# LiWentomng/OrientedRepPoints

Measured on AMD Instinct MI355X. Metric: images/sec (1024x1024 DOTA, R-50 FPN), higher is better.
Workload: dtype f32; 1 GPU; configs[1]: OrientedRepPoints R-50 FPN inference, 1024x1024 patch, 15 classes, bs=1/GPU, nms_pre=2000, score_thr=0.05, rnms iou_thr=0.4, max_per_img=2000; random-init weights, head biases calibrated to ~2000 dets/img; global_batch=1, parallelism=replicas x1 (image-parallel, no collective), images_in_flight_per_gpu=4

## Files before the change

### include/orp_hip.h

```cpp
#ifndef ORP_HIP_H_
#define ORP_HIP_H_

#include <stddef.h>
#include <stdint.h>

#ifdef __cplusplus
extern "C" {
#endif

#define ORP_OK 0
#define ORP_EINVAL (-1)
#define ORP_EWORKSPACE (-2)
#define ORP_ETOOBIG (-3)

const char* orp_version(void);

#define ORP_NMS_MAX_BOXES 131072
size_t orp_rnms_workspace_bytes(int n);
int orp_rnms(const float* dets, int n, float iou_thr, int flavor, int presorted, int order_out,
             int64_t* keep_out, int32_t* num_keep, void* workspace, size_t workspace_bytes, void* stream);

size_t orp_rnms_batched_workspace_bytes(int n_total, int nseg, int max_seg);
int orp_rnms_batched(const float* dets, int n_total, const int32_t* seg_offsets, int nseg, int max_seg,
                     float iou_thr, int flavor, int64_t* keep_out, int32_t* num_keep,
// ... 226 lines not shown
int orp_fpn_topdown_nhwc(const orp_norm_level* levels, const float* const* gammas_host, const float* const* betas_host,
                         int nlevels, int batch, int channels, int groups, float eps, uint32_t* amax_out, void* workspace,
                         size_t workspace_bytes, void* stream);

typedef struct { const float* input; const float* residual; float* output; float* output2; int height; int width; } orp_bias_level;
int orp_bias_act_multi(const orp_bias_level* levels_host, int nlevels, int batch, int channels, const float* bias,
                       const float* sub, int relu, void* stream);

size_t orp_conv1x1_packed_floats(int c_in);
int orp_conv1x1_ok(int c_in, int c_out);
int orp_conv1x1_pack_weight(const float* weight, int c_out, int c_in, float* packed, void* stream);
int orp_conv1x1_multi(const orp_bias_level* levels_host, int nlevels, int batch, int c_in, int c_out,
                      const float* weight_packed, const float* bias, const float* sub, int relu, void* stream);

int orp_conv1x1_bn_act_ok(int c_in, int c_out);
int orp_conv1x1_bn_act_pays(int c_in, int c_out, int hw, int batch, int has_residual);
int orp_conv1x1_bn_act_tile(int c_in, int c_out, int hw, int batch, int* tile_channels, int* tile_positions);
int orp_conv1x1_bn_act(const float* x, const float* weight_t, const float* scale, const float* shift, const float* residual,
                       const float* scale2, const float* shift2, float* y, int batch, int c_in, int c_out, int hw, int relu,
                       void* stream);

int orp_conv1x1_bn_act_range(const float* x, const float* weight_t, const float* scale, const float* shift, const float* residual,
                             const float* scale2, const float* shift2, float* y, int batch, int c_in, int c_out, int hw, int relu,
                             uint32_t* range_out, void* stream);
int orp_conv1x1_bn_act_pieces_ok(int c_in, int c_out);
int orp_conv1x1_bn_act_pieces_pays(int c_in, int c_out, int hw, int batch, int has_residual);
int orp_conv1x1_bn_act_pieces_tile(int c_in, int c_out, int hw, int batch, int* tile_channels, int* tile_positions);
size_t orp_conv1x1_bn_pieces_packed_bytes(int c_in, int c_out);
int orp_conv1x1_bn_pieces_pack_weight(const float* weight, int c_in, int c_out, void* packed, void* stream);
int orp_conv1x1_bn_act_pieces(const float* x, const void* weight_packed, const float* scale, const float* shift,
                              const float* residual, const float* scale2, const float* shift2, float* y, int batch, int c_in,
                              int c_out, int hw, int relu, uint32_t* range_out, void* stream);

int orp_conv1x1_bn_act_pieces_dual_ok(int c_in, int c_in2, int c_out);
int orp_conv1x1_bn_act_pieces_dual_pays(int c_in, int c_in2, int c_out, int hw, int stride2, int batch);
int orp_conv1x1_bn_act_pieces_dual_tile(int c_in, int c_in2, int c_out, int hw, int batch, int* tile_channels, int* tile_positions);
int orp_conv1x1_bn_act_pieces_dual(const float* x, const void* w_packed, const float* scale, const float* shift, const float* x2,
                                   const void* w2_packed, const float* scale2, const float* shift2, int c_in2, int h2, int w2,
                                   int stride2, float* y, int batch, int c_in, int c_out, int ho, int wo, int relu, void* stream);

int orp_affine_act_range(const float* x, const float* residual, const float* scale, const float* shift, float* y, int batch,
                         int channels, int hw, int relu, uint32_t* range_out, void* stream);

int orp_conv3x3_bn_act_ok(int c_in, int c_out);
int orp_conv3x3_bn_act_pays(int c_in, int c_out, int height, int width, int batch);
int orp_conv3x3_bn_act_tile(int c_in, int c_out, int height, int width, int batch, int* tile_h, int* tile_w, int* waves_pos,
                            int* waves_ch);
size_t orp_conv3x3_bn_packed_bytes(int c_in, int c_out);
int orp_conv3x3_bn_pack_weight(const float* weight, int c_in, int c_out, void* packed, void* stream);
int orp_conv3x3_bn_act(const float* x, const void* weight_packed, const float* scale, const float* shift, const uint32_t* range_in,
                       float* y, int batch, int c_in, int c_out, int height, int width, int relu, void* stream);

int orp_conv3x3_bn_deep_ok(int c_in, int c_out, int stride);
int orp_conv3x3_bn_deep_pays(int c_in, int c_out, int height, int width, int stride, int batch);
size_t orp_conv3x3_bn_deep_packed_bytes(int c_in, int c_out);
int orp_conv3x3_bn_deep_pack_weight(const float* weight, int c_in, int c_out, void* packed, void* stream);
int orp_conv3x3_bn_deep(const float* x, const void* weight_packed, const float* scale, const float* shift, const uint32_t* range_in,
                        float* y, int batch, int c_in, int c_out, int height, int width, int stride, int relu, void* stream);


int orp_conv3x3_small_ok(int c_in, int c_out);
int orp_conv3x3_small_multi(const orp_norm_level* levels_host, int nlevels, int batch, int c_in, int c_out,
                            const float* weight_packed, void* stream);
int orp_conv3x3_small_multi_ex(const orp_norm_level* levels_host, const float* const* weights_packed_host, int nlevels,
                               int batch, int c_in, int c_out, void* stream);
size_t orp_conv3x3_small_workspace_bytes(const orp_norm_level* levels_host, const int* strides_host, int nlevels, int batch,
// ... 94 lines not shown
```

### orientedreppoints_amd/_lib.py

```python
import ctypes
import os

import torch

_HERE = os.path.dirname(os.path.abspath(__file__))
LIB_PATH = os.environ.get("ORP_HIP_LIB") or os.path.join(_HERE, "csrc", "liborp_hip.so")

ORP_OK, ORP_EINVAL, ORP_EWORKSPACE, ORP_ETOOBIG = 0, -1, -2, -3
ORP_NMS_MAX_BOXES = 131072

_vp = ctypes.c_void_p
_i = ctypes.c_int
_f = ctypes.c_float
_sz = ctypes.c_size_t

_SIGNATURES = {
    "orp_version": (ctypes.c_char_p, []),
    "orp_rnms_workspace_bytes": (_sz, [_i]),
    "orp_rnms": (_i, [_vp, _i, _f, _i, _i, _i, _vp, _vp, _vp, _sz, _vp]),
    "orp_rnms_batched_workspace_bytes": (_sz, [_i, _i, _i]),
    "orp_rnms_batched": (_i, [_vp, _i, _vp, _i, _i, _f, _i, _vp, _vp, _vp, _sz, _vp]),
    "_poly_nms": (None, [_vp, _vp, _vp, _i, _i, _f, _i]),
    "_overlaps": (None, [_vp, _vp, _vp, _i, _i, _i]),
    "orp_quad_iou_matrix": (_i, [_vp, _i, _vp, _i, _i, _i, _vp, _vp]),
# ... 57 lines not shown
    "orp_poly_nms_f64_workspace_bytes": (_sz, [_i]),
    "orp_poly_nms_f64": (_i, [_vp, _i, ctypes.c_double, _vp, _vp, _vp, _sz, _vp]),
    "orp_poly_nms_f64_batched_workspace_bytes": (_sz, [_i, _i, _i]),
    "orp_poly_nms_f64_batched": (_i, [_vp, _i, _vp, _i, _i, ctypes.c_double, _i, _i, _vp, _vp, _vp, _sz, _vp]),
    "orp_scene_tiles": (_i, [_vp, _i, _i, ctypes.c_longlong, _vp, _i, _i, _vp, _vp, _i, _i, _vp, _vp]),
    "orp_scene_tiles_resized": (_i, [_vp, _i, _i, ctypes.c_longlong, _vp, _i, _i, _i, _i, _i, _i, _i, _vp, _vp, _vp, _vp, _vp, _vp, _i,
                                     _i, _vp, _vp]),
    "orp_scene_tiles_flip": (_i, [_vp, _i, _i, ctypes.c_longlong, _vp, _i, _i, _vp, _vp, _i, _i, _vp, _vp]),
    "orp_scene_tiles_resized_flip": (_i, [_vp, _i, _i, ctypes.c_longlong, _vp, _i, _i, _i, _i, _i, _i, _i, _vp, _vp, _vp, _vp, _vp,
                                          _vp, _i, _i, _vp, _vp]),
    "orp_scene_collect_workspace_bytes": (_sz, [_i, _i]),
    "orp_scene_collect": (_i, [_vp, _i, _i, _vp, ctypes.c_double, _i, _i, _vp, _vp, _vp, _vp, _vp, _sz, _vp]),
    "orp_soft_rnms_host": (_i, [_vp, _i, _f, _i, _f, _f, _vp, _vp]),
    "orp_conv1x1_packed_floats": (_sz, [_i]),
    "orp_conv1x1_ok": (_i, [_i, _i]),
    "orp_conv1x1_pack_weight": (_i, [_vp, _i, _i, _vp, _vp]),
    "orp_conv1x1_multi": (_i, [_vp, _i, _i, _i, _i, _vp, _vp, _vp, _i, _vp]),
    "orp_conv1x1_bn_act_ok": (_i, [_i, _i]),
    "orp_conv1x1_bn_act_pays": (_i, [_i, _i, _i, _i, _i]),
    "orp_conv1x1_bn_act_tile": (_i, [_i, _i, _i, _i, _vp, _vp]),
    "orp_conv1x1_bn_act": (_i, [_vp, _vp, _vp, _vp, _vp, _vp, _vp, _vp, _i, _i, _i, _i, _i, _vp]),
    "orp_conv1x1_bn_act_range": (_i, [_vp, _vp, _vp, _vp, _vp, _vp, _vp, _vp, _i, _i, _i, _i, _i, _vp, _vp]),
    "orp_affine_act_range": (_i, [_vp, _vp, _vp, _vp, _vp, _i, _i, _i, _i, _vp, _vp]),
    "orp_conv1x1_bn_act_pieces_ok": (_i, [_i, _i]),
    "orp_conv1x1_bn_act_pieces_pays": (_i, [_i, _i, _i, _i, _i]),
    "orp_conv1x1_bn_act_pieces_tile": (_i, [_i, _i, _i, _i, _vp, _vp]),
    "orp_conv1x1_bn_pieces_packed_bytes": (_sz, [_i, _i]),
    "orp_conv1x1_bn_pieces_pack_weight": (_i, [_vp, _i, _i, _vp, _vp]),
    "orp_conv1x1_bn_act_pieces": (_i, [_vp, _vp, _vp, _vp, _vp, _vp, _vp, _vp, _i, _i, _i, _i, _i, _vp, _vp]),
    "orp_conv1x1_bn_act_pieces_dual_ok": (_i, [_i, _i, _i]),
    "orp_conv1x1_bn_act_pieces_dual_pays": (_i, [_i, _i, _i, _i, _i, _i]),
    "orp_conv1x1_bn_act_pieces_dual_tile": (_i, [_i, _i, _i, _i, _i, _vp, _vp]),
    "orp_conv1x1_bn_act_pieces_dual": (_i, [_vp, _vp, _vp, _vp, _vp, _vp, _vp, _vp, _i, _i, _i, _i, _vp, _i, _i, _i, _i, _i, _i, _vp]),
    "orp_conv3x3_bn_act_ok": (_i, [_i, _i]),
    "orp_conv3x3_bn_act_pays": (_i, [_i, _i, _i, _i, _i]),
    "orp_conv3x3_bn_act_tile": (_i, [_i, _i, _i, _i, _i, _vp, _vp, _vp, _vp]),
    "orp_conv3x3_bn_packed_bytes": (_sz, [_i, _i]),
    "orp_conv3x3_bn_pack_weight": (_i, [_vp, _i, _i, _vp, _vp]),
    "orp_conv3x3_bn_act": (_i, [_vp, _vp, _vp, _vp, _vp, _vp, _i, _i, _i, _i, _i, _i, _vp]),
    "orp_conv3x3_bn_deep_ok": (_i, [_i, _i, _i]),
    "orp_conv3x3_bn_deep_pays": (_i, [_i, _i, _i, _i, _i, _i]),
    "orp_conv3x3_bn_deep_packed_bytes": (_sz, [_i, _i]),
    "orp_conv3x3_bn_deep_pack_weight": (_i, [_vp, _i, _i, _vp, _vp]),
    "orp_conv3x3_bn_deep": (_i, [_vp, _vp, _vp, _vp, _vp, _vp, _i, _i, _i, _i, _i, _i, _i, _vp]),
    "orp_pp_select_scratch_bytes": (_sz, [_i, _i, _i]),
    "orp_pp_select": (_i, [_vp, _i, _i, _vp, _i, _i, _vp, _vp, _sz, _vp]),
    "orp_pp_gather": (_i, [_vp, _vp, _i, _i, _vp, _vp, _vp, _i, _vp, _vp, _vp, _vp, _vp]),
    "orp_pp_compact_scratch_bytes": (_sz, [_i]),
    "orp_pp_compact": (_i, [_vp, _vp, _i, _i, _i, _vp, _f, _i, _vp, _vp, _vp, _vp, _vp, _vp, _sz, _vp]),
    "orp_pp_compact_views_scratch_bytes": (_sz, [_i]),
    "orp_pp_compact_views": (_i, [_vp, _i, _i, _f, _i, _vp, _vp, _vp, _vp, _vp, _vp, _vp, _vp, _sz, _vp]),
    "orp_pp_pack": (_i, [_vp, _vp, _vp, _vp, _vp, _vp, _vp, _vp, _i, _i, _vp, _vp]),
    "orp_groupnorm_workspace_bytes": (_sz, [_vp, _i, _i, _i, _i]),
    "orp_groupnorm_act_multi": (_i, [_vp, _i, _i, _i, _i, _vp, _vp, _f, _i, _vp, _sz, _vp]),
    "orp_groupnorm_act_multi_ex": (_i, [_vp, _vp, _vp, _i, _i, _i, _i, _f, _i, _vp, _sz, _vp]),
    "orp_groupnorm_act_multi_nhwc": (_i, [_vp, _vp, _vp, _vp, _i, _i, _i, _i, _f, _i, _vp, _sz, _vp]),
    "orp_groupnorm_act_multi_train": (_i, [_vp, _vp, _vp, _i, _i, _i, _i, _f, _i, _vp, _vp, _sz, _vp]),
    "orp_groupnorm_backward_workspace_bytes": (_sz, [_vp, _i, _i, _i, _i]),
    "orp_groupnorm_act_multi_backward": (_i, [_vp, _vp, _vp, _vp, _vp, _vp, _vp, _i, _i, _i, _i, _i, _vp, _vp, _sz, _vp]),
    "orp_voc_best_match_f64": (_i, [_vp, _vp, _i, _vp, _vp, _i, _vp, _vp, _vp]),
    "orp_affine_act": (_i, [_vp, _vp, _vp, _vp, _vp, _i, _i, _i, _i, _vp]),
    "orp_affine2_act": (_i, [_vp, _vp, _vp, _vp, _vp, _vp, _vp, _i, _i, _i, _i, _vp]),
    "orp_affine_relu_maxpool": (_i, [_vp, _vp, _vp, _vp, _i, _i, _i, _i, _vp]),
    "orp_fpn_topdown_workspace_bytes": (_sz, [_vp, _i, _i, _i, _i]),
    "orp_fpn_topdown_nhwc": (_i, [_vp, _vp, _vp, _i, _i, _i, _i, _f, _vp, _vp, _sz, _vp]),
    "orp_bias_act_multi": (_i, [_vp, _i, _i, _i, _vp, _vp, _i, _vp]),
# ... 105 lines not shown
```

### orientedreppoints_amd/build.py

```python
import concurrent.futures
import os
import subprocess

HERE = os.path.dirname(os.path.abspath(__file__))
CSRC = os.path.join(HERE, "csrc")
LIB = os.path.join(CSRC, "liborp_hip.so")
HIPCC = os.environ.get("HIPCC", "/opt/rocm/bin/hipcc")
ARCH = "gfx950"

NO_PACKED_FP32 = ["-Xclang", "-target-feature", "-Xclang", "-packed-fp32-ops"]
COMMON = ["--offload-arch=" + ARCH, "-O3", "-std=c++17", "-fPIC", "-Wall", "-Wno-unused-function",
          "-Wno-unused-result", "-Wno-unused-value",
          "-Wno-bitwise-instead-of-logical"]
if os.environ.get("ORP_PACKED_FP32", "0") != "1":
    COMMON = COMMON + NO_PACKED_FP32
SOURCES = [
    ("orp_nms.hip", ["-ffp-contract=off"]),
    ("orp_overlaps.hip", ["-ffp-contract=off"]),
    ("orp_minarearect.hip", ["-ffp-contract=off"]),
    ("orp_box_iou_rotated.hip", ["-ffp-contract=off"]),
    ("orp_convex.hip", ["-ffp-contract=off"]),
    ("orp_convex_giou.hip", ["-ffp-contract=off"]),
    ("orp_pointwise.hip", ["-ffp-contract=off"]),
    ("orp_assign.hip", ["-ffp-contract=off"]),
    ("orp_postproc.hip", ["-ffp-contract=off"]),
    ("orp_soft_rnms.hip", ["-ffp-contract=off"]),
    ("orp_scene.hip", ["-ffp-contract=off"]),
    ("orp_eval.hip", ["-ffp-contract=off"]),
    ("orp_train.hip", ["-ffp-contract=off"]),
    ("orp_norm.hip", []),
    ("orp_conv_small.hip", []),
    ("orp_conv1x1.hip", []),
    ("orp_conv1x1_bn.hip", []),
    ("orp_conv1x1_bn_pieces.hip", []),
    ("orp_conv3x3_bn.hip", []),
    ("orp_conv3x3_bn_deep.hip", []),
    ("orp_dcn.hip", []),
    ("orp_dcn_split.hip", ["-ffp-contract=off"]),
    ("orp_conv_split.hip", []),
    ("orp_conv_wgrad.hip", []),
    ("orp_dcn_half.hip", []),
    ("orp_dcn_bwd.hip", []),
    ("orp_dcn_bwd_mfma.hip", []),
    ("orp_window_attn.hip", []),
    ("orp_prof.hip", []),
]
HEADERS = ["orp_affine.hpp", "orp_geom.hpp", "orp_quadfast.hpp", "orp_tile.hpp", "orp_hull.hpp", "orp_libm.hpp", "orp_prof.hpp", "orp_launch.hpp", "orp_dcn_split.hpp", "orp_dcn_common.hpp", "orp_range.hpp", "orp_conv1x1_bn_host.hpp", os.path.join("..", "..", "include", "orp_hip.h")]


def _stale(target, deps):
    if not os.path.exists(target):
        return True
    t = os.path.getmtime(target)
    return any(os.path.getmtime(d) > t for d in deps if os.path.exists(d))


VERSION_SOURCE = "orp_overlaps.hip"


def build_id():
    import hashlib
    h = hashlib.sha1()
    names = sorted([s for s, _ in SOURCES] + [x for x in HEADERS])
    for n in names:
        path = os.path.join(CSRC, n)
        if os.path.exists(path):
            h.update(n.encode())
# ... 44 lines not shown
```

### orientedreppoints_amd/mmdet_models/resnet.py

```python
import torch
import torch.nn as nn

from .. import switches
from .layers import build_conv_layer, build_norm_layer, constant_init, kaiming_init
from .registry import BACKBONES


class Bottleneck(nn.Module):
    expansion = 4

    def __init__(self, inplanes, planes, stride=1, dilation=1, downsample=None, style='pytorch',
                 norm_cfg=dict(type='BN'), dcn=None):
        super(Bottleneck, self).__init__()
        assert style in ['pytorch', 'caffe']
        assert dcn is None or isinstance(dcn, dict)
        if style == 'pytorch':
            conv1_stride, conv2_stride = 1, stride
        else:
            conv1_stride, conv2_stride = stride, 1
        self.conv1 = nn.Conv2d(inplanes, planes, kernel_size=1, stride=conv1_stride, bias=False)
        self.add_module('bn1', build_norm_layer(norm_cfg, planes)[1])
        self.with_dcn = dcn is not None
        fallback_on_stride = False
        if self.with_dcn:
            fallback_on_stride = dcn.pop('fallback_on_stride', False)
            dcn = dict(dcn)
            if 'modulated' in dcn:
                dcn.setdefault('type', 'DCNv2' if dcn.pop('modulated') else 'DCN')
            dcn.setdefault('type', 'DCN')
        use_dcn = self.with_dcn and not fallback_on_stride
        self.conv2 = build_conv_layer(dcn if use_dcn else None, planes, planes, kernel_size=3, stride=conv2_stride,
                                      padding=dilation, dilation=dilation, bias=False)
        self.conv2_is_dcn = use_dcn
        self.add_module('bn2', build_norm_layer(norm_cfg, planes)[1])
        self.conv3 = nn.Conv2d(planes, planes * self.expansion, kernel_size=1, bias=False)
        self.add_module('bn3', build_norm_layer(norm_cfg, planes * self.expansion)[1])
        self.relu = nn.ReLU(inplace=True)
        self.downsample = downsample

    def _fused_ok(self, x):
        return (not torch.is_grad_enabled()) and x.is_cuda and x.dtype == torch.float32 and \
            isinstance(self.bn1, nn.BatchNorm2d) and not self.bn1.training and not self.bn3.training

    def _downsample_norm_fusable(self):
        return switches.of(self, 'fuse_downsample_norm', 'BN_DOWNSAMPLE_FUSE') and self._downsample_is_conv_norm()

    def _downsample_is_conv_norm(self):
        ds = self.downsample
        return isinstance(ds, nn.Sequential) and len(ds) == 2 and isinstance(ds[0], nn.Conv2d) and \
            isinstance(ds[1], nn.BatchNorm2d) and not ds[1].training

    def _conv1x1_fusable(self):
        return switches.of(self, 'fuse_conv1x1', 'BN_CONV1X1_FUSE')

    def _conv1x1_pieces_on(self):
        return switches.of(self, 'fuse_conv1x1_pieces', 'BN_CONV1X1_PIECES')

    def _downsample_conv_fusable(self):
        return switches.of(self, 'fuse_downsample_conv', 'BN_DOWNSAMPLE_CONV_FUSE')

    def _conv3x3_fusable(self):
        return switches.of(self, 'fuse_conv3x3', 'BN_CONV3X3_FUSE') and not self.conv2_is_dcn and \
            isinstance(self.bn2, nn.BatchNorm2d) and not self.bn2.training

    def _conv3x3_deep_fusable(self):
        return switches.of(self, 'fuse_conv3x3_deep', 'BN_CONV3X3_DEEP_FUSE') and not self.conv2_is_dcn and \
            isinstance(self.bn2, nn.BatchNorm2d) and not self.bn2.training

    def _forward_fused(self, x):
        from ..mmdet_ops.fused_norm import bn_act, conv1x1_bn_act, conv3x3_bn_act, conv3x3_bn_act_routed, \
            conv3x3_bn_deep, conv3x3_bn_deep_routed, conv1x1_bn_act_dual, conv1x1_bn_act_dual_routed
        fuse = self._conv1x1_fusable()
        pieces = None if self._conv1x1_pieces_on() else False

        def conv_bn_act(t, conv, bn, **kw):
            if fuse:
                return conv1x1_bn_act(t, conv, bn, pieces=pieces, **kw)
            return bn_act(conv(t).contiguous(), bn, **kw)
        force3 = bool(getattr(self, 'force_conv3x3', False))
        fuse3 = False
        if self._conv3x3_fusable() and tuple(self.conv1.stride) == (1, 1):
            fuse3 = conv3x3_bn_act_routed(x, self.conv2, self.bn2, force3,
                                          shape=(x.size(0), self.conv1.out_channels, x.size(2), x.size(3)))
        force3d = bool(getattr(self, 'force_conv3x3_deep', False))
        deep3 = False
        if not fuse3 and self._conv3x3_deep_fusable() and tuple(self.conv1.stride) == (1, 1):
            deep3 = conv3x3_bn_deep_routed(x, self.conv2, self.bn2, force3d,
                                           shape=(x.size(0), self.conv1.out_channels, x.size(2), x.size(3)))
        if fuse3:
            out, bits = conv_bn_act(x, self.conv1, self.bn1, relu=True, want_range=True)
            out = conv3x3_bn_act(out, self.conv2, self.bn2, relu=True, force=force3, range_bits=bits)
        elif deep3:
            out, bits = conv_bn_act(x, self.conv1, self.bn1, relu=True, want_range=True)
            out = conv3x3_bn_deep(out, self.conv2, self.bn2, relu=True, force=force3d, range_bits=bits)
        else:
            out = conv_bn_act(x, self.conv1, self.bn1, relu=True)
            out = bn_act(self.conv2(out).contiguous(), self.bn2, relu=True)
        ds = self.downsample
        if fuse and pieces is None and self._downsample_conv_fusable() and self._downsample_is_conv_norm() and \
                conv1x1_bn_act_dual_routed(out, self.conv3, self.bn3, x, ds[0], ds[1]):
            return conv1x1_bn_act_dual(out, self.conv3, self.bn3, x, ds[0], ds[1], relu=True)
        if self._downsample_norm_fusable():
            residual, residual_bn = ds[0](x).contiguous(), ds[1]
        elif ds is not None:
            residual, residual_bn = bn_act(ds[0](x).contiguous(), ds[1], relu=False), None
        else:
            residual, residual_bn = x.contiguous(), None
        return conv_bn_act(out, self.conv3, self.bn3, residual=residual, residual_bn=residual_bn, relu=True)

    def forward(self, x):
# ... 138 lines not shown
```

### orientedreppoints_amd/mmdet_ops/fused_norm.py

```python
import ctypes

import torch

from .. import _lib, _packcache


class _NormLevel(ctypes.Structure):
    _fields_ = [("input", ctypes.c_void_p), ("output", ctypes.c_void_p), ("height", ctypes.c_int),
                ("width", ctypes.c_int)]


def _call(name, device, *args):
    with torch.cuda.device(device):
        rc = getattr(_lib.lib(), name)(*args)
    _lib.check(rc, name)


def _norm_levels(ins, outs):
    levels = (_NormLevel * len(ins))()
    for i, (x, y) in enumerate(zip(ins, outs)):
        levels[i] = _NormLevel(x.data_ptr(), y.data_ptr() if y is not None else None, x.size(2), x.size(3))
    return levels


# ... 177 lines not shown

def conv1x1_bn_act_ok(x, conv, bn):
    w = conv.weight
    return bool(isinstance(conv, torch.nn.Conv2d) and _bn_input(x, bn) and x.dim() == 4 and
                _plain_conv(conv, w, 1, ((1, 1),), 0) and x.size(1) == w.size(1) and x.size(2) * x.size(3) > 0 and
                _lib.lib().orp_conv1x1_bn_act_ok(w.size(1), w.size(0)))


_packed_1x1_pieces = _packcache.new_cache("conv1x1_bn_pieces_weight")


def _packed_1x1_planes(weight):
    return _packed_planes(_packed_1x1_pieces, weight, "orp_conv1x1_bn_pieces_packed_bytes", "orp_conv1x1_bn_pieces_pack_weight",
                          lambda w: w.float().reshape(w.size(0), w.size(1)).contiguous())


def conv1x1_bn_act_pieces_tile(cin, cout, hw, B):
    return _tile_query("orp_conv1x1_bn_act_pieces_tile", 2, cin, cout, hw, B)


def _conv1x1_route(shape, force, pieces):
    if shape is None:
        return None
    L = _lib.lib()
    if not (force and pieces is None) and pieces is not False:
        if pieces is None:
            from .. import switches
            pieces = bool(switches.BN_CONV1X1_PIECES) and bool(L.orp_conv1x1_bn_act_pieces_pays(*shape))
        if bool(pieces) and bool(L.orp_conv1x1_bn_act_pieces_ok(shape[0], shape[1])):
            return 'pieces'
    return 'fp32' if force or bool(L.orp_conv1x1_bn_act_pays(*shape)) else None


def conv1x1_bn_act(x, conv, bn, residual=None, residual_bn=None, relu=True, force=False, want_range=False, pieces=None):
    if residual_bn is not None and residual is None:
        raise ValueError("conv1x1_bn_act: residual_bn without a residual")
    if want_range and residual is not None:
        raise ValueError("conv1x1_bn_act: want_range with a residual")
    fused = conv1x1_bn_act_ok(x, conv, bn) and (residual_bn is None or not residual_bn.training)
    shape = (x.size(1), conv.weight.size(0), x.size(2) * x.size(3), x.size(0), 1 if residual is not None else 0) if fused else None
    route = _conv1x1_route(shape, force, pieces)
    if route is None:
        return bn_act(conv(x).contiguous(), bn, residual=residual, relu=relu, residual_bn=residual_bn, want_range=want_range)
    x = x.detach().contiguous()
    B, cin, H, W = x.shape
    cout = conv.weight.size(0)
    if residual is not None:
        residual = residual.detach()
        if not (tuple(residual.shape) == (B, cout, H, W) and residual.is_contiguous() and residual.dtype == torch.float32):
            raise ValueError("conv1x1_bn_act: residual must be a contiguous fp32 tensor of the output's shape")
    weight = _packed_1x1_planes(conv.weight) if route == 'pieces' else _transposed_1x1_weight(conv.weight)
    scale, shift = _bn_affine(bn)
    scale2, shift2 = _bn_affine(residual_bn) if residual_bn is not None else (None, None)
    y = torch.empty((B, cout, H, W), dtype=torch.float32, device=x.device)
    bits = torch.empty(1, dtype=torch.int32, device=x.device) if want_range else None
    args = (_lib.ptr(x), _lib.ptr(weight), _lib.ptr(scale), _lib.ptr(shift), _lib.ptr(residual), _lib.ptr(scale2), _lib.ptr(shift2),
            _lib.ptr(y), B, cin, cout, H * W, 1 if relu else 0)
    if route == 'pieces':
        _call("orp_conv1x1_bn_act_pieces", x.device, *args, _lib.ptr(bits), _lib.stream_of(x))
    elif want_range:
        _call("orp_conv1x1_bn_act_range", x.device, *args, _lib.ptr(bits), _lib.stream_of(x))
    else:
        _call("orp_conv1x1_bn_act", x.device, *args, _lib.stream_of(x))
    return (y, bits) if want_range else y


def conv1x1_bn_act_dual_ok(x, conv, bn, x2, conv2, bn2):
    if not conv1x1_bn_act_ok(x, conv, bn):
        return False
    w2 = getattr(conv2, 'weight', None)
    if not (isinstance(conv2, torch.nn.Conv2d) and _bn_input(x2, bn2) and x2.dim() == 4 and x2.device == x.device and
            _plain_conv(conv2, w2, 1, ((1, 1), (2, 2)), 0) and x2.size(1) == w2.size(1) and
            w2.size(0) == conv.weight.size(0) and x2.size(0) == x.size(0)):
        return False
    s = conv2.stride[0]
    return bool(x2.size(2) > 0 and x2.size(3) > 0 and (x2.size(2) - 1) // s + 1 == x.size(2) and (x2.size(3) - 1) // s + 1 == x.size(3)
                and _lib.lib().orp_conv1x1_bn_act_pieces_dual_ok(conv.weight.size(1), w2.size(1), w2.size(0)))


def conv1x1_bn_act_dual_pays(x, conv, x2, conv2):
    return bool(_lib.lib().orp_conv1x1_bn_act_pieces_dual_pays(conv.weight.size(1), conv2.weight.size(1), conv.weight.size(0),
                                                               x.size(2) * x.size(3), conv2.stride[0], x.size(0)))


def conv1x1_bn_act_dual_routed(x, conv, bn, x2, conv2, bn2):
    return conv1x1_bn_act_dual_ok(x, conv, bn, x2, conv2, bn2) and conv1x1_bn_act_dual_pays(x, conv, x2, conv2)


def conv1x1_bn_act_dual_tile(cin, cin2, cout, hw, B):
    return _tile_query("orp_conv1x1_bn_act_pieces_dual_tile", 2, cin, cin2, cout, hw, B)

# ... 712 lines not shown
```

### orientedreppoints_amd/switches.py

```python
import os


def _on(name, default='1'):
    return os.environ.get(name, default) == '1'


TOWER_SPLIT = _on('ORP_TOWER_SPLIT')
FPN_SPLIT = _on('ORP_FPN_SPLIT')
TOWER_GN_FUSE = _on('ORP_TOWER_GN_FUSE')
BN_DOWNSAMPLE_FUSE = _on('ORP_BN_DOWNSAMPLE_FUSE')
BN_CONV1X1_FUSE = _on('ORP_BN_CONV1X1_FUSE')
BN_CONV1X1_PIECES = _on('ORP_BN_CONV1X1_PIECES')
BN_DOWNSAMPLE_CONV_FUSE = _on('ORP_BN_DOWNSAMPLE_CONV_FUSE')
BN_CONV3X3_FUSE = _on('ORP_BN_CONV3X3_FUSE')
BN_CONV3X3_DEEP_FUSE = _on('ORP_BN_CONV3X3_DEEP_FUSE')
STEM_POOL_FUSE = _on('ORP_STEM_POOL_FUSE')
SWIN_ATTN_FUSE = _on('ORP_SWIN_ATTN_FUSE')
SWIN_ATTN_TRAIN_FUSE = _on('ORP_SWIN_ATTN_TRAIN_FUSE')
SWIN_ATTN_HALF_FUSE = _on('ORP_SWIN_ATTN_HALF_FUSE')
FPN_TOPDOWN_FUSE = _on('ORP_FPN_TOPDOWN_FUSE')
TRAIN_SPLIT = _on('ORP_TRAIN_SPLIT')
DETERMINISTIC = _on('ORP_DETERMINISTIC', '0')


def of(obj, attr, name):
    on = getattr(obj, attr, None)
    return bool(globals()[name] if on is None else on)
```

Measured before the change: 431.4 images/s.

## Add split-K deep 1x1 conv+BN kernel for wide-input layers

Adds a new fused 1x1 conv+BN+act HIP kernel. Each workgroup of eight waves splits the input-channel reduction across K groups and sums the partial results through LDS, which reuses the staging buffer. It keeps the three-plane bf16 split of the fp32 inputs on 32x32x16 MFMA and double-buffers the staged activations. The route is enabled by default but only taken where the pays table lists the shape (2048->512 channels at 32x32, batch 1), targeting the low-occupancy deep ResNet stage. The cost is an extra LDS reduction pass and a larger kernel and build surface.

Measured after the change: 431.4 images/s. No clear change (-0.0%).

```diff
diff --git a/include/orp_hip.h b/include/orp_hip.h
--- a/include/orp_hip.h
+++ b/include/orp_hip.h
@@ -282,6 +282,17 @@
                               const float* residual, const float* scale2, const float* shift2, float* y, int batch, int c_in,
                               int c_out, int hw, int relu, uint32_t* range_out, void* stream);
 
+int orp_conv1x1_bn_deep_ok(int c_in, int c_out);
+int orp_conv1x1_bn_deep_pays(int c_in, int c_out, int hw, int batch);
+int orp_conv1x1_bn_deep_tile(int c_in, int c_out, int hw, int batch, int* tile_channels, int* tile_positions, int* k_groups);
+int orp_conv1x1_bn_deep(const float* x, const void* weight_packed, const float* scale, const float* shift, float* y, int batch,
+                        int c_in, int c_out, int hw, int relu, uint32_t* range_out, void* stream);
+int orp_conv1x1_bn_deep_layouts(void);
+int orp_conv1x1_bn_deep_layout_info(int layout, int* tile_channels, int* tile_positions, int* k_groups, int* k_step);
+int orp_conv1x1_bn_deep_layout_of(int c_in, int c_out);
+int orp_conv1x1_bn_deep_at(int layout, const float* x, const void* weight_packed, const float* scale, const float* shift, float* y,
+                           int batch, int c_in, int c_out, int hw, int relu, uint32_t* range_out, void* stream);
+
 int orp_conv1x1_bn_act_pieces_dual_ok(int c_in, int c_in2, int c_out);
 int orp_conv1x1_bn_act_pieces_dual_pays(int c_in, int c_in2, int c_out, int hw, int stride2, int batch);
 int orp_conv1x1_bn_act_pieces_dual_tile(int c_in, int c_in2, int c_out, int hw, int batch, int* tile_channels, int* tile_positions);
diff --git a/orientedreppoints_amd/_lib.py b/orientedreppoints_amd/_lib.py
--- a/orientedreppoints_amd/_lib.py
+++ b/orientedreppoints_amd/_lib.py
@@ -113,6 +113,14 @@
     "orp_conv1x1_bn_act_pieces_dual_pays": (_i, [_i, _i, _i, _i, _i, _i]),
     "orp_conv1x1_bn_act_pieces_dual_tile": (_i, [_i, _i, _i, _i, _i, _vp, _vp]),
     "orp_conv1x1_bn_act_pieces_dual": (_i, [_vp, _vp, _vp, _vp, _vp, _vp, _vp, _vp, _i, _i, _i, _i, _vp, _i, _i, _i, _i, _i, _i, _vp]),
+    "orp_conv1x1_bn_deep_ok": (_i, [_i, _i]),
+    "orp_conv1x1_bn_deep_pays": (_i, [_i, _i, _i, _i]),
+    "orp_conv1x1_bn_deep_tile": (_i, [_i, _i, _i, _i, _vp, _vp, _vp]),
+    "orp_conv1x1_bn_deep": (_i, [_vp, _vp, _vp, _vp, _vp, _i, _i, _i, _i, _i, _vp, _vp]),
+    "orp_conv1x1_bn_deep_layouts": (_i, []),
+    "orp_conv1x1_bn_deep_layout_info": (_i, [_i, _vp, _vp, _vp, _vp]),
+    "orp_conv1x1_bn_deep_layout_of": (_i, [_i, _i]),
+    "orp_conv1x1_bn_deep_at": (_i, [_i, _vp, _vp, _vp, _vp, _vp, _i, _i, _i, _i, _i, _vp, _vp]),
     "orp_conv3x3_bn_act_ok": (_i, [_i, _i]),
     "orp_conv3x3_bn_act_pays": (_i, [_i, _i, _i, _i, _i]),
     "orp_conv3x3_bn_act_tile": (_i, [_i, _i, _i, _i, _i, _vp, _vp, _vp, _vp]),
diff --git a/orientedreppoints_amd/build.py b/orientedreppoints_amd/build.py
--- a/orientedreppoints_amd/build.py
+++ b/orientedreppoints_amd/build.py
@@ -33,6 +33,7 @@
     ("orp_conv1x1.hip", []),
     ("orp_conv1x1_bn.hip", []),
     ("orp_conv1x1_bn_pieces.hip", []),
+    ("orp_conv1x1_bn_deep.hip", []),
     ("orp_conv3x3_bn.hip", []),
     ("orp_conv3x3_bn_deep.hip", []),
     ("orp_dcn.hip", []),
diff --git a/orientedreppoints_amd/csrc/orp_conv1x1_bn_deep.hip b/orientedreppoints_amd/csrc/orp_conv1x1_bn_deep.hip
--- /dev/null
+++ b/orientedreppoints_amd/csrc/orp_conv1x1_bn_deep.hip
@@ -0,0 +1,381 @@
+#include <hip/hip_runtime.h>
+#include <stdint.h>
+#include <type_traits>
+
+#include "../../include/orp_hip.h"
+#include "orp_affine.hpp"
+#include "orp_range.hpp"
+#include "orp_launch.hpp"
+#include "orp_conv1x1_bn_host.hpp"
+
+namespace {
+
+constexpr int kThreads = 512;
+
+typedef float f32x16 __attribute__((ext_vector_type(16)));
+typedef __bf16 bf8 __attribute__((ext_vector_type(8)));
+
+struct Args {
+  const float* x;
+  const uint16_t* planes;
+  size_t plane_stride;
+  const float* scale; const float* shift;
+  const float* res; const float* scale2; const float* shift2;
+  float* y;
+  int cin, cout, hw, relu;
+  int ntm, ntn;
+  unsigned* range;
+  int xs, ptiles;
+};
+
+__device__ __forceinline__ unsigned pack_hi16(float a, float b) {
+  return __builtin_amdgcn_perm(__float_as_uint(b), __float_as_uint(a), 0x07060302u);
+}
+
+__device__ __forceinline__ void split_pair(float a, float b, unsigned (&d)[3]) {
+  const float a0 = __uint_as_float(__float_as_uint(a) & 0xffff0000u), b0 = __uint_as_float(__float_as_uint(b) & 0xffff0000u);
+  const float ar = a - a0, br = b - b0;
+  const float a1 = __uint_as_float(__float_as_uint(ar) & 0xffff0000u), b1 = __uint_as_float(__float_as_uint(br) & 0xffff0000u);
+  d[0] = pack_hi16(a0, b0);
+  d[1] = pack_hi16(a1, b1);
+  d[2] = pack_hi16(ar - a1, br - b1);
+}
+
+template <int WCH_, int KG_, int WN_, int BK_>
+struct Cfg {
+  static constexpr int WCH = WCH_, KG = KG_, WN = WN_, BK = BK_;
+  static_assert(WCH * KG == kThreads / 64, "eight waves");
+  static constexpr int ASTR = BK + 8;
+  static constexpr int NCH = BK / 16;
+  static constexpr int BM = 32 * WCH, BN = 32 * WN;
+  static constexpr int PLANE = BN * ASTR, GBUF = 3 * PLANE, BUF = KG * GBUF;
+  static constexpr int GITEMS = (BK / 2) * (BN / 4);
+  static constexpr int XV = KG * GITEMS / kThreads;
+  static_assert(KG * GITEMS % kThreads == 0 && XV >= 1, "every thread stages XV whole items per K step");
+  static constexpr size_t stage_bytes = (size_t)2 * BUF * 2;
+  static constexpr size_t smem = stage_bytes + (size_t)2 * BM * sizeof(float) + 8 * sizeof(unsigned);
+  static_assert(smem <= 163840, "a workgroup may take 160 KiB of LDS");
+  static constexpr int RG = WCH * WN * 16 * 64;
+  static_assert((size_t)(KG - 1) * RG * sizeof(float) <= stage_bytes, "the reduction reuses the staging area");
+};
+
+template <class K, bool VEC, bool RANGE>
+__global__ void __launch_bounds__(kThreads)
+conv1x1_bn_deep_kernel(const Args P) {
+  constexpr int WCH = K::WCH, KG = K::KG, WN = K::WN, BK = K::BK;
+  constexpr int ASTR = K::ASTR, NCH = K::NCH, BM = K::BM, BN = K::BN, PLANE = K::PLANE, GBUF = K::GBUF, BUF = K::BUF, XV = K::XV;
+  extern __shared__ __attribute__((aligned(16))) unsigned char smem[];
+  uint16_t* lds = reinterpret_cast<uint16_t*>(smem);
+  float* Cs = reinterpret_cast<float*>(smem + K::stage_bytes);
+  unsigned* rred = reinterpret_cast<unsigned*>(Cs + 2 * BM);
+
+  const int tid = threadIdx.x;
+  const int xcd = blockIdx.x & 7, j = blockIdx.x >> 3;
+  const int ntg = P.ntm / P.xs;
+  const int mt = (xcd % P.xs) * ntg + j % ntg;
+  const int pt = (j / ntg) * (8 / P.xs) + xcd / P.xs;
+  if (pt >= P.ptiles) return;
+  const int nt = pt % P.ntn, b = pt / P.ntn;
+  const int m0 = mt * BM, p0 = nt * BN;
+  const int hw = P.hw, cout = P.cout;
+  const int slice = P.cin / KG;
+  const float* xb = P.x + (size_t)b * P.cin * hw;
+  if (tid < BM) {
+    const int ch = min(m0 + tid, cout - 1);
+    Cs[tid] = P.scale[ch]; Cs[BM + tid] = P.shift[ch];
+  }
+
+  const int lane = tid & 63, wave = tid >> 6;
+  const int kg = lane >> 5, l31 = lane & 31;
+  const int wc = wave % WCH, g = wave / WCH;
+  const int wm0 = wc * 32;
+
+  const size_t wblk = (size_t)2 * cout * 8;
+  const uint16_t* wp = P.planes + ((size_t)kg * cout + min(m0 + wm0 + l31, cout - 1)) * 8 + (size_t)(g * (slice / 16)) * wblk;
+  bf8 wq[NCH][3];
+  auto load_w = [&](int t, int c) {
+    const uint16_t* a = wp + (size_t)(t * NCH + c) * wblk;
+#pragma unroll
+    for (int pl = 0; pl < 3; pl++) wq[c][pl] = *reinterpret_cast<const bf8*>(a + (size_t)pl * P.plane_stride);
+  };
+#pragma unroll
+  for (int c = 0; c < NCH; c++) load_w(0, c);
+
+  float4 xr[2][XV][2];
+  int xpq[XV], xkp[XV], xg[XV];
+#pragma unroll
+  for (int i = 0; i < XV; i++) {
+    const int idx = tid + i * kThreads;
+    xg[i] = idx / K::GITEMS;
+    const int loc = idx % K::GITEMS;
+    xpq[i] = loc & (BN / 4 - 1);
+    xkp[i] = loc / (BN / 4);
+  }
+  auto fetch = [&](int k0, float4 (&xr)[XV][2]) {
+#pragma unroll
+    for (int i = 0; i < XV; i++) {
+      const int col = p0 + 4 * xpq[i];
+#pragma unroll
+      for (int h = 0; h < 2; h++) {
+        const float* src = xb + (size_t)(xg[i] * slice + k0 + 2 * xkp[i] + h) * hw;
+        if (VEC) {
+          xr[i][h] = *reinterpret_cast<const float4*>(src + min(col, hw - 4));
+        } else {
+          xr[i][h].x = src[min(col, hw - 1)]; xr[i][h].y = src[min(col + 1, hw - 1)];
+          xr[i][h].z = src[min(col + 2, hw - 1)]; xr[i][h].w = src[min(col + 3, hw - 1)];
+        }
+      }
+    }
+  };
+  auto stage = [&](int buf, const float4 (&xr)[XV][2]) {
+#pragma unroll
+    for (int i = 0; i < XV; i++) {
+      const int col = p0 + 4 * xpq[i];
+      float v[2][4];
+#pragma unroll
+      for (int h = 0; h < 2; h++) {
+        v[h][0] = col < hw ? xr[i][h].x : 0.f; v[h][1] = col + 1 < hw ? xr[i][h].y : 0.f;
+        v[h][2] = col + 2 < hw ? xr[i][h].z : 0.f; v[h][3] = col + 3 < hw ? xr[i][h].w : 0.f;
+      }
+      const int rot = (xpq[i] >> 1) & 3;
+#pragma unroll
+      for (int h = 0; h < 2; h++) {
+        if (rot & 1) { const float t0 = v[h][0]; v[h][0] = v[h][1]; v[h][1] = v[h][2]; v[h][2] = v[h][3]; v[h][3] = t0; }
+        if (rot & 2) { const float t0 = v[h][0], t1 = v[h][1]; v[h][0] = v[h][2]; v[h][1] = v[h][3]; v[h][2] = t0; v[h][3] = t1; }
+      }
+      unsigned* base = reinterpret_cast<unsigned*>(lds + buf * BUF + xg[i] * GBUF) + xkp[i];
+#pragma unroll
+      for (int j = 0; j < 4; j++) {
+        unsigned d[3];
+        split_pair(v[0][j], v[1][j], d);
+        unsigned* dst = base + (4 * xpq[i] + ((j + rot) & 3)) * (ASTR / 2);
+#pragma unroll
+        for (int pl = 0; pl < 3; pl++) dst[pl * (PLANE / 2)] = d[pl];
+      }
+    }
+  };
+
+  f32x16 acc[WN];
+#pragma unroll
+  for (int ni = 0; ni < WN; ni++)
+#pragma unroll
+    for (int r = 0; r < 16; r++) acc[ni][r] = 0.f;
+
+  auto mma = [&](int buf, int t_next) {
+    const uint16_t* xa = lds + buf * BUF + g * GBUF + l31 * ASTR + 8 * kg;
+    auto load_x = [&](int c, bf8 (&q)[WN][3]) {
+#pragma unroll
+      for (int ni = 0; ni < WN; ni++)
+#pragma unroll
+        for (int pl = 0; pl < 3; pl++) q[ni][pl] = *reinterpret_cast<const bf8*>(xa + pl * PLANE + ni * 32 * ASTR + c * 16);
+    };
+    bf8 xqs[2][WN][3];
+    load_x(0, xqs[0]);
+#pragma unroll
+    for (int c = 0; c < NCH; c++) {
+      bf8 (&xq)[WN][3] = xqs[c & 1];
+      if (c + 1 < NCH) load_x(c + 1, xqs[(c + 1) & 1]);
+      __builtin_amdgcn_sched_barrier(0);
+#pragma unroll
+      for (int ni = 0; ni < WN; ni++) acc[ni] = __builtin_amdgcn_mfma_f32_32x32x16_bf16(wq[c][0], xq[ni][2], acc[ni], 0, 0, 0);
+#pragma unroll
+      for (int ni = 0; ni < WN; ni++) acc[ni] = __builtin_amdgcn_mfma_f32_32x32x16_bf16(wq[c][2], xq[ni][0], acc[ni], 0, 0, 0);
+#pragma unroll
+      for (int ni = 0; ni < WN; ni++) acc[ni] = __builtin_amdgcn_mfma_f32_32x32x16_bf16(wq[c][1], xq[ni][1], acc[ni], 0, 0, 0);
+#pragma unroll
+      for (int ni = 0; ni < WN; ni++) acc[ni] = __builtin_amdgcn_mfma_f32_32x32x16_bf16(wq[c][0], xq[ni][1], acc[ni], 0, 0, 0);
+#pragma unroll
+      for (int ni = 0; ni < WN; ni++) acc[ni] = __builtin_amdgcn_mfma_f32_32x32x16_bf16(wq[c][1], xq[ni][0], acc[ni], 0, 0, 0);
+#pragma unroll
+      for (int ni = 0; ni < WN; ni++) acc[ni] = __builtin_amdgcn_mfma_f32_32x32x16_bf16(wq[c][0], xq[ni][0], acc[ni], 0, 0, 0);
+      __builtin_amdgcn_sched_barrier(0);
+      load_w(t_next, c);
+      __builtin_amdgcn_sched_barrier(0);
+    }
+  };
+
+  const int nk = slice / BK;
+  auto step = [&](int t, float4 (&cur)[XV][2], float4 (&nxt)[XV][2], int buf) {
+    fetch(min(t + 2, nk - 1) * BK, cur);
+    __builtin_amdgcn_sched_barrier(0);
+    mma(buf, t + 1);
+    stage(buf ^ 1, nxt);
+    __syncthreads();
+  };
+  fetch(0, xr[0]);
+  stage(0, xr[0]);
+  fetch(min(1, nk - 1) * BK, xr[1]);
+  __syncthreads();
+  int t = 0;
+  for (; t + 2 < nk; t += 2) {
+    step(t, xr[0], xr[1], 0);
+    step(t + 1, xr[1], xr[0], 1);
+  }
+  if (t + 1 < nk) step(t, xr[0], xr[1], 0);
+  mma((nk - 1) & 1, nk - 1);
+
+  float* red = reinterpret_cast<float*>(smem) + (size_t)wc * WN * 16 * 64 + lane;
+  __syncthreads();
+  if (g > 0) {
+#pragma unroll
+    for (int ni = 0; ni < WN; ni++)
+#pragma unroll
+      for (int r = 0; r < 16; r++) red[(g - 1) * K::RG + (ni * 16 + r) * 64] = acc[ni][r];
+  }
+  __syncthreads();
+
+  unsigned rmax = 0u;
+  if (g == 0) {
+    const size_t plane0 = (size_t)b * cout;
+#pragma unroll
+    for (int q4 = 0; q4 < 4; q4++) {
+      const int chg = m0 + wm0 + 8 * q4 + 4 * kg;
+      const float* cs = Cs + wm0 + 8 * q4 + 4 * kg;
+      const float4 a4 = *reinterpret_cast<const float4*>(cs);
+      const float4 b4 = *reinterpret_cast<const float4*>(cs + BM);
+      const float av[4] = {a4.x, a4.y, a4.z, a4.w}, bv[4] = {b4.x, b4.y, b4.z, b4.w};
+#pragma unroll
+      for (int ni = 0; ni < WN; ni++) {
+        const int p = p0 + 32 * ni + l31;
+#pragma unroll
+        for (int q = 0; q < 4; q++) {
+          const int r = 4 * q4 + q;
+          float v = acc[ni][r];
+#pragma unroll
+          for (int k = 0; k < KG - 1; k++) v += red[k * K::RG + (ni * 16 + r) * 64];
+          const float o = affine_act(v, av[q], bv[q], P.relu);
+          if (chg < cout && p < hw) {
+            P.y[(plane0 + chg + q) * hw + p] = o;
+            if (RANGE) rmax = max(rmax, orp::range_bits(o));
+          }
+        }
+      }
+    }
+  }
+  if (RANGE) {
+#pragma unroll
+    for (int o = 32; o > 0; o >>= 1) rmax = max(rmax, (unsigned)__shfl_xor((int)rmax, o, 64));
+    if (g == 0 && lane == 0) rred[wc] = rmax;
+    __syncthreads();
+    if (tid == 0) {
+      unsigned m = rred[0];
+#pragma unroll
+      for (int i = 1; i < WCH; i++) m = max(m, rred[i]);
+      orp::range_raise(P.range, m);
+    }
+  }
+}
+
+using orp_c1x1::Tile;
+
+using L0 = Cfg<2, 4, 2, 32>;
+using L1 = Cfg<2, 4, 1, 64>;
+using L2 = Cfg<4, 2, 1, 64>;
+constexpr int kLayouts = 3;
+struct LayoutInfo { int bm, bn, kg, bk; };
+constexpr LayoutInfo kInfo[kLayouts] = {{L0::BM, L0::BN, L0::KG, L0::BK}, {L1::BM, L1::BN, L1::KG, L1::BK}, {L2::BM, L2::BN, L2::KG, L2::BK}};
+
+int layout_of(int c_in, int c_out) {
+  if (c_in == 1024 && (c_out == 256 || c_out == 512)) return 2;
+  return 1;
+}
+
+bool layout_takes(int layout, int c_in, int c_out) {
+  if (layout < 0 || layout >= kLayouts) return false;
+  const LayoutInfo& I = kInfo[layout];
+  return c_in >= I.kg * I.bk && c_in <= 2048 && c_in % (I.kg * I.bk) == 0 && c_out >= 64 && c_out <= 4096 && c_out % 32 == 0;
+}
+
+template <class K>
+Tile tile_of(int, int, int) { return Tile{K::BM, K::BN}; }
+
+template <class K, bool VEC, bool RANGE>
+struct LdsTag {};
+
+long grid_order(Args& A, int batch) {
+  int xs = 1;
+  while (xs < 8 && A.ntm % (2 * xs) == 0 && (size_t)6 * A.cin * A.cout / xs > ((size_t)2 << 20)) xs *= 2;
+  A.xs = xs;
+  const long pt = (long)A.ntn * batch;
+  A.ptiles = (int)pt;
+  const int per = 8 / xs;
+  return 8L * (A.ntm / xs) * ((pt + per - 1) / per);
+}
+
+template <class K>
+void launch(Args& A, int batch, bool vec, hipStream_t st) {
+  const long wgs = grid_order(A, batch);
+  if (wgs >= (1L << 31)) return;
+  auto go = [&](auto range, auto v) {
+    auto fn = &conv1x1_bn_deep_kernel<K, decltype(v)::value, decltype(range)::value>;
+    using Tag = LdsTag<K, decltype(v)::value, decltype(range)::value>;
+    if (orp::set_max_dynamic_lds_once<Tag>(reinterpret_cast<const void*>(fn), K::smem) != hipSuccess) return;
+    hipLaunchKernelGGL(fn, dim3((unsigned)wgs), dim3(kThreads), K::smem, st, A);
+  };
+  if (A.range) { if (vec) go(std::true_type{}, std::true_type{}); else go(std::true_type{}, std::false_type{}); }
+  else { if (vec) go(std::false_type{}, std::true_type{}); else go(std::false_type{}, std::false_type{}); }
+}
+
+int run_layout(int layout, const float* x, const void* weight_packed, const float* scale, const float* shift, float* y, int batch,
+               int c_in, int c_out, int hw, int relu, uint32_t* range_out, void* stream) {
+  Tile (*pick[kLayouts])(int, int, int) = {tile_of<L0>, tile_of<L1>, tile_of<L2>};
+  const bool ok = layout_takes(layout, c_in, c_out);
+  return orp_c1x1::run<Args>(x, weight_packed, scale, shift, nullptr, nullptr, nullptr, y, batch, c_in, c_out, hw, relu, range_out, stream,
+                             ok, pick[ok ? layout : 0], [&](Args& A, Tile, bool vec, hipStream_t st) {
+    A.planes = reinterpret_cast<const uint16_t*>(weight_packed); A.plane_stride = (size_t)c_in * c_out;
+    if (layout == 0) launch<L0>(A, batch, vec, st);
+    else if (layout == 1) launch<L1>(A, batch, vec, st);
+    else launch<L2>(A, batch, vec, st);
+  });
+}
+
+}
+
+extern "C" {
+
+int orp_conv1x1_bn_deep_ok(int c_in, int c_out) {
+  return (c_in >= 256 && c_in <= 2048 && c_in % 256 == 0 && c_out >= 64 && c_out <= 4096 && c_out % 32 == 0) ? 1 : 0;
+}
+
+int orp_conv1x1_bn_deep_tile(int c_in, int c_out, int hw, int batch, int* tile_channels, int* tile_positions, int* k_groups) {
+  if (!orp_conv1x1_bn_deep_ok(c_in, c_out) || hw <= 0 || batch <= 0) return 0;
+  const LayoutInfo& I = kInfo[layout_of(c_in, c_out)];
+  if (tile_channels) *tile_channels = I.bm;
+  if (tile_positions) *tile_positions = I.bn;
+  if (k_groups) *k_groups = I.kg;
+  return 1;
+}
+
+int orp_conv1x1_bn_deep_layouts(void) { return kLayouts; }
+int orp_conv1x1_bn_deep_layout_info(int layout, int* tile_channels, int* tile_positions, int* k_groups, int* k_step) {
+  if (layout < 0 || layout >= kLayouts) return 0;
+  const LayoutInfo& I = kInfo[layout];
+  if (tile_channels) *tile_channels = I.bm;
+  if (tile_positions) *tile_positions = I.bn;
+  if (k_groups) *k_groups = I.kg;
+  if (k_step) *k_step = I.bk;
+  return 1;
+}
+int orp_conv1x1_bn_deep_layout_of(int c_in, int c_out) { return orp_conv1x1_bn_deep_ok(c_in, c_out) ? layout_of(c_in, c_out) : -1; }
+
+int orp_conv1x1_bn_deep_pays(int c_in, int c_out, int hw, int batch) {
+  if (!orp_conv1x1_bn_deep_ok(c_in, c_out) || hw <= 0 || batch <= 0) return 0;
+  static const orp_c1x1::PaidRow paid[] = {
+      {2048, 512, 1024, 1024, 1},
+  };
+  return orp_c1x1::paid(paid, c_in, c_out, hw, batch);
+}
+
+int orp_conv1x1_bn_deep(const float* x, const void* weight_packed, const float* scale, const float* shift, float* y, int batch, int c_in,
+                        int c_out, int hw, int relu, uint32_t* range_out, void* stream) {
+  if (!orp_conv1x1_bn_deep_ok(c_in, c_out)) return ORP_EINVAL;
+  return run_layout(layout_of(c_in, c_out), x, weight_packed, scale, shift, y, batch, c_in, c_out, hw, relu, range_out, stream);
+}
+
+int orp_conv1x1_bn_deep_at(int layout, const float* x, const void* weight_packed, const float* scale, const float* shift, float* y,
+                           int batch, int c_in, int c_out, int hw, int relu, uint32_t* range_out, void* stream) {
+  if (!layout_takes(layout, c_in, c_out)) return ORP_EINVAL;
+  return run_layout(layout, x, weight_packed, scale, shift, y, batch, c_in, c_out, hw, relu, range_out, stream);
+}
+
+}
diff --git a/orientedreppoints_amd/mmdet_models/resnet.py b/orientedreppoints_amd/mmdet_models/resnet.py
--- a/orientedreppoints_amd/mmdet_models/resnet.py
+++ b/orientedreppoints_amd/mmdet_models/resnet.py
@@ -56,6 +56,9 @@
     def _conv1x1_pieces_on(self):
         return switches.of(self, 'fuse_conv1x1_pieces', 'BN_CONV1X1_PIECES')
 
+    def _conv1x1_deep_on(self):
+        return switches.of(self, 'fuse_conv1x1_deep', 'BN_CONV1X1_DEEP')
+
     def _downsample_conv_fusable(self):
         return switches.of(self, 'fuse_downsample_conv', 'BN_DOWNSAMPLE_CONV_FUSE')
 
@@ -72,10 +75,12 @@
             conv3x3_bn_deep, conv3x3_bn_deep_routed, conv1x1_bn_act_dual, conv1x1_bn_act_dual_routed
         fuse = self._conv1x1_fusable()
         pieces = None if self._conv1x1_pieces_on() else False
+        deep = self._conv1x1_deep_on()
+        force1d = bool(getattr(self, 'force_conv1x1_deep', False))
 
         def conv_bn_act(t, conv, bn, **kw):
             if fuse:
-                return conv1x1_bn_act(t, conv, bn, pieces=pieces, **kw)
+                return conv1x1_bn_act(t, conv, bn, pieces=pieces, deep=deep, force_deep=force1d, **kw)
             return bn_act(conv(t).contiguous(), bn, **kw)
         force3 = bool(getattr(self, 'force_conv3x3', False))
         fuse3 = False
diff --git a/orientedreppoints_amd/mmdet_ops/fused_norm.py b/orientedreppoints_amd/mmdet_ops/fused_norm.py
--- a/orientedreppoints_amd/mmdet_ops/fused_norm.py
+++ b/orientedreppoints_amd/mmdet_ops/fused_norm.py
@@ -233,14 +233,31 @@
     return 'fp32' if force or bool(L.orp_conv1x1_bn_act_pays(*shape)) else None
 
 
-def conv1x1_bn_act(x, conv, bn, residual=None, residual_bn=None, relu=True, force=False, want_range=False, pieces=None):
+def conv1x1_bn_deep_tile(cin, cout, hw, B):
+    return _tile_query("orp_conv1x1_bn_deep_tile", 3, cin, cout, hw, B)
+
+
+def _conv1x1_deep_route(shape, force, pieces, deep, force_deep):
+    if shape is None or shape[4] or force or pieces is not None:
+        return False
+    if deep is None:
+        from .. import switches
+        deep = switches.BN_CONV1X1_DEEP
+    if not deep:
+        return False
+    L = _lib.lib()
+    return bool(L.orp_conv1x1_bn_deep_ok(shape[0], shape[1])) and bool(force_deep or L.orp_conv1x1_bn_deep_pays(*shape[:4]))
+
+
+def conv1x1_bn_act(x, conv, bn, residual=None, residual_bn=None, relu=True, force=False, want_range=False, pieces=None, deep=None,
+                   force_deep=False):
     if residual_bn is not None and residual is None:
         raise ValueError("conv1x1_bn_act: residual_bn without a residual")
     if want_range and residual is not None:
         raise ValueError("conv1x1_bn_act: want_range with a residual")
     fused = conv1x1_bn_act_ok(x, conv, bn) and (residual_bn is None or not residual_bn.training)
     shape = (x.size(1), conv.weight.size(0), x.size(2) * x.size(3), x.size(0), 1 if residual is not None else 0) if fused else None
-    route = _conv1x1_route(shape, force, pieces)
+    route = 'deep' if _conv1x1_deep_route(shape, force, pieces, deep, force_deep) else _conv1x1_route(shape, force, pieces)
     if route is None:
         return bn_act(conv(x).contiguous(), bn, residual=residual, relu=relu, residual_bn=residual_bn, want_range=want_range)
     x = x.detach().contiguous()
@@ -250,14 +267,17 @@
         residual = residual.detach()
         if not (tuple(residual.shape) == (B, cout, H, W) and residual.is_contiguous() and residual.dtype == torch.float32):
             raise ValueError("conv1x1_bn_act: residual must be a contiguous fp32 tensor of the output's shape")
-    weight = _packed_1x1_planes(conv.weight) if route == 'pieces' else _transposed_1x1_weight(conv.weight)
+    weight = _packed_1x1_planes(conv.weight) if route in ('pieces', 'deep') else _transposed_1x1_weight(conv.weight)
     scale, shift = _bn_affine(bn)
     scale2, shift2 = _bn_affine(residual_bn) if residual_bn is not None else (None, None)
     y = torch.empty((B, cout, H, W), dtype=torch.float32, device=x.device)
     bits = torch.empty(1, dtype=torch.int32, device=x.device) if want_range else None
     args = (_lib.ptr(x), _lib.ptr(weight), _lib.ptr(scale), _lib.ptr(shift), _lib.ptr(residual), _lib.ptr(scale2), _lib.ptr(shift2),
             _lib.ptr(y), B, cin, cout, H * W, 1 if relu else 0)
-    if route == 'pieces':
+    if route == 'deep':
+        _call("orp_conv1x1_bn_deep", x.device, _lib.ptr(x), _lib.ptr(weight), _lib.ptr(scale), _lib.ptr(shift), _lib.ptr(y), B, cin, cout,
+              H * W, 1 if relu else 0, _lib.ptr(bits), _lib.stream_of(x))
+    elif route == 'pieces':
         _call("orp_conv1x1_bn_act_pieces", x.device, *args, _lib.ptr(bits), _lib.stream_of(x))
     elif want_range:
         _call("orp_conv1x1_bn_act_range", x.device, *args, _lib.ptr(bits), _lib.stream_of(x))
diff --git a/orientedreppoints_amd/switches.py b/orientedreppoints_amd/switches.py
--- a/orientedreppoints_amd/switches.py
+++ b/orientedreppoints_amd/switches.py
@@ -11,6 +11,7 @@
 BN_DOWNSAMPLE_FUSE = _on('ORP_BN_DOWNSAMPLE_FUSE')
 BN_CONV1X1_FUSE = _on('ORP_BN_CONV1X1_FUSE')
 BN_CONV1X1_PIECES = _on('ORP_BN_CONV1X1_PIECES')
+BN_CONV1X1_DEEP = _on('ORP_BN_CONV1X1_DEEP')
 BN_DOWNSAMPLE_CONV_FUSE = _on('ORP_BN_DOWNSAMPLE_CONV_FUSE')
 BN_CONV3X3_FUSE = _on('ORP_BN_CONV3X3_FUSE')
 BN_CONV3X3_DEEP_FUSE = _on('ORP_BN_CONV3X3_DEEP_FUSE')
```
